# zhoujoey/ORB-SLAM3-Mac

Hardware: AMD Instinct MI355X
Metric: ORB extract+match frames/sec (higher is better)
Workload: dtype u8; 1 GPU; vga: synthetic 640x480 batch=1024 per GPU, 8-level pyramid, 1000 feats/frame, ORB extract + Hamming 2-NN match (Frame.cc:1146) + SearchForInitialization (ORBmatcher.cc:710) vs successor frame; pipelines=1, matchers=side by side (two contexts), frames_total=1024

## Files before the change

include/orbhip.h:

```cpp
#ifndef ORBHIP_H
#define ORBHIP_H
#include <stddef.h>
#include <stdint.h>
#ifdef __cplusplus
extern "C" {
#endif

#define ORBHIP_OK 0
#define ORBHIP_E_BADARG (-1)
#define ORBHIP_E_NODEVICE (-2)
#define ORBHIP_E_HIP (-3)
#define ORBHIP_E_CAPACITY (-4)
#define ORBHIP_E_ABORTED (-5)
#define ORBHIP_E_NOTSPD (-6)
#define ORBHIP_E_EMPTY (-7)

typedef struct {
    float x, y, size, angle, response;
    int32_t octave, class_id;
} orbhip_keypoint;

typedef struct orbhip_ctx orbhip_ctx;
typedef struct orbhip_extractor orbhip_extractor;

const char *orbhip_version(void);
const char *orbhip_last_error(void);

int orbhip_ctx_create(int device, void *stream, orbhip_ctx **out);
void orbhip_ctx_destroy(orbhip_ctx *ctx);
int orbhip_ctx_synchronize(orbhip_ctx *ctx);
int orbhip_ctx_wait_for(orbhip_ctx *ctx, orbhip_ctx *other);
int orbhip_ctx_check_status(orbhip_ctx *ctx);
void *orbhip_ctx_stream(orbhip_ctx *ctx);

int orbhip_extractor_create(orbhip_ctx *ctx, int nfeatures, float scale_factor, int nlevels,
                            int ini_th_fast, int min_th_fast, orbhip_extractor **out);
void orbhip_extractor_destroy(orbhip_extractor *ext);

int orbhip_extractor_levels(const orbhip_extractor *ext);
int orbhip_extractor_table(const orbhip_extractor *ext, int which, float *out);
int orbhip_extractor_features_per_level(const orbhip_extractor *ext, int *out);
int orbhip_extractor_umax(const orbhip_extractor *ext, int *out16);

int orbhip_extractor_reserve(orbhip_extractor *ext, int width, int height, int max_batch);
int orbhip_extractor_max_keypoints(const orbhip_extractor *ext);

int orbhip_extract_batch_device(orbhip_extractor *ext, const uint8_t *d_images, int width,
                                int height, size_t row_stride, size_t frame_stride, int batch,
                                int lap0, int lap1);
int orbhip_extractor_results(orbhip_extractor *ext, orbhip_keypoint **d_kp, uint8_t **d_desc,
                             int32_t **d_count, int32_t **d_mono_index);
int orbhip_extract_batch_host(orbhip_extractor *ext, const uint8_t *h_images, int width, int height,
                              size_t row_stride, size_t frame_stride, int batch, int lap0, int lap1,
                              orbhip_keypoint *kp_out, uint8_t *desc_out, int cap,
                              int32_t *count_out, int32_t *mono_out);
int orbhip_extract_batch_host_view(orbhip_extractor *ext, const uint8_t *h_images, int width, int height, size_t row_stride,
                                   size_t frame_stride, int batch, int lap0, int lap1, const orbhip_keypoint **kp_view,
                                   const uint8_t **desc_view, int *row_capacity, const int32_t **count_view, const int32_t **mono_view);
int orbhip_extractor_blur_kernel(const orbhip_extractor *ext, int batch);

int orbhip_extractor_resize_band_rows(const orbhip_extractor *ext, int level);

int orbhip_extractor_last_frame(orbhip_extractor *ext, int frame, const orbhip_keypoint **d_kp, const uint8_t **d_desc,
                                const orbhip_keypoint **h_kp_view, const uint8_t **h_desc_view, int32_t *count, unsigned long long *generation);

int orbhip_extractor_level_dims(const orbhip_extractor *ext, int level, int *w, int *h);
int orbhip_extractor_get_pyramid_level(orbhip_extractor *ext, int frame, int level, int padded,
                                       uint8_t *h_out, size_t out_stride);
int orbhip_extractor_get_pyramid_padded(orbhip_extractor *ext, int frame, uint8_t *const *levels_out, const size_t *strides);
int orbhip_extractor_get_blurred_level(orbhip_extractor *ext, int frame, int level,
                                       uint8_t *h_out, size_t out_stride);
int orbhip_extractor_get_fast_candidates(orbhip_extractor *ext, int frame, int level,
                                         int32_t *xs, int32_t *ys, int32_t *scores, int cap,
                                         int32_t *n_out);
int orbhip_extractor_get_level_keypoints(orbhip_extractor *ext, int frame, int level,
                                         orbhip_keypoint *out, int cap, int32_t *n_out);

int orbhip_extractor_set_graph_mode(orbhip_extractor *ext, int enable);

#define ORBHIP_STAGE_PYRAMID 0
#define ORBHIP_STAGE_FAST_CELLS 1
#define ORBHIP_STAGE_BLUR 2
#define ORBHIP_STAGE_OCTREE 3
#define ORBHIP_STAGE_DESC 4
#define ORBHIP_STAGE_ASSEMBLE 5
#define ORBHIP_STAGE_COUNT 6
int orbhip_extractor_set_profiling(orbhip_extractor *ext, int enable);
int orbhip_extractor_stage_ms(orbhip_extractor *ext, float *ms_out );

int orbhip_descriptor_distance(const uint8_t *a32, const uint8_t *b32);

int orbhip_match_bf2nn_device(orbhip_ctx *ctx, const uint8_t *d_descA, const int32_t *d_nA,
                              size_t strideA, const uint8_t *d_descB, const int32_t *d_nB,
                              size_t strideB, int pairs, int max_n, double ratio,
                              int32_t *d_idx2, int32_t *d_dist2, uint8_t *d_accept);

int orbhip_search_for_initialization_device(orbhip_ctx *ctx,
        const orbhip_keypoint *d_kpA, const uint8_t *d_descA, const int32_t *d_nA,
        const orbhip_keypoint *d_kpB, const uint8_t *d_descB, const int32_t *d_nB,
        int pairs, int max_n, size_t frame_stride_kp , float min_x, float min_y,
        float max_x, float max_y, int window_size, float nn_ratio, int check_orientation,
        float *d_prev_matched, int32_t *d_matches12, int32_t *d_nmatches);

int orbhip_prev_matched_init_device(orbhip_ctx *ctx, const orbhip_keypoint *d_kp, size_t frame_stride_kp,
                                    int frames, int max_n, float *d_prev_matched);

typedef struct orbhip_proj_query {
    float u, v, radius, ur, angle;
    int32_t min_level, max_level, has_obs;
} orbhip_proj_query;
int orbhip_search_by_projection_device(orbhip_ctx *ctx, const orbhip_proj_query *d_q, const uint8_t *d_desc_q,
                                       const int32_t *d_nq, int max_q, const orbhip_keypoint *d_kp,
                                       const uint8_t *d_desc, const float *d_u_right, const int32_t *d_n, int max_n,
                                       size_t frame_stride_kp, int pairs, float min_x, float min_y, float max_x,
                                       float max_y, int th_high, int check_orientation, int32_t *d_train_match,
                                       int32_t *d_nmatches);

int orbhip_search_local_map_device(orbhip_ctx *ctx, const orbhip_proj_query *d_q, const uint8_t *d_desc_q,
                                   const int32_t *d_nq, int max_q, const orbhip_keypoint *d_kp,
                                   const uint8_t *d_desc, const float *d_u_right, const int32_t *d_n, int max_n,
                                   size_t frame_stride_kp, int pairs, float min_x, float min_y, float max_x,
                                   float max_y, int th_high, float nn_ratio, int32_t *d_train_match,
                                   int32_t *d_nmatches);

int orbhip_search_by_projection_rig_device(orbhip_ctx *ctx, int mode, const orbhip_proj_query *d_q, const uint8_t *d_desc_q,
                                           const int32_t *d_nq, int max_q, const orbhip_keypoint *d_kp, const uint8_t *d_desc,
                                           const int32_t *d_n, const int32_t *d_nleft, const int32_t *d_mirror, int max_n,
                                           size_t frame_stride_kp, int pairs, float min_x, float min_y, float max_x, float max_y,
                                           int th_high, float nn_ratio, int check_orientation, int32_t *d_train_match,
// ... 398 lines not shown
```

orb-slam3-mac_amd/csrc/orb_kernels.hip:

```cpp
#include "orb_internal.h"
#include "wave_dpp.h"
#include <mutex>
#include <vector>
#include <cstdio>
#include <cstdlib>

#define WAVE 64

__device__ __forceinline__ int wave_incl_scan(int v) { return wave_scan_add_dpp(v); }

__device__ __forceinline__ int block_excl_scan256(int v, int *wsum, int *total)
{
    const int lane = threadIdx.x & (WAVE - 1), wid = threadIdx.x >> 6;
    int inc = wave_incl_scan(v);
    if (lane == WAVE - 1) wsum[wid] = inc;
    __syncthreads();
    int base = 0;
#pragma unroll
    for (int w = 0; w < 4; w++) {
        int s = wsum[w];
        if (w < wid) base += s;
    }
    *total = wsum[0] + wsum[1] + wsum[2] + wsum[3];
    __syncthreads();
// ... 754 lines not shown
    const long fair = total / (8 * nblocks);
    const int cmax = runs ? 8 : 4;
    F.chunk = chunk_env > 0 ? chunk_env : (int)(fair < 1 ? 1 : fair > cmax ? cmax : fair);
    if (runs && nld == 4) hipLaunchKernelGGL(k_fast_runs<4>, dim3((unsigned)nblocks), dim3(64), lds, s, F);
    else if (runs) hipLaunchKernelGGL(k_fast_runs<6>, dim3((unsigned)nblocks), dim3(64), lds, s, F);
    else if (F.small_cells) hipLaunchKernelGGL((k_fast_cells<3, 24, 2>), dim3((unsigned)nblocks), dim3(64), lds, s, F);
    else hipLaunchKernelGGL((k_fast_cells<5, 32, 5>), dim3((unsigned)nblocks), dim3(64), lds, s, F);
}
const void *orb_fast_cells_func(int small) { return small ? reinterpret_cast<const void *>(k_fast_cells<3, 24, 2>) : reinterpret_cast<const void *>(k_fast_cells<5, 32, 5>); }

struct OctLds {
    uint32_t *cc;
    int *ord;
    int *by_ord;
    int *excl;
    int *posbase;
    int *newpos;
    uint32_t *best;
};

int orb_octree_nc(const OrbParams &P)
{
    int nc = 0;
    for (int l = 0; l < P.nlevels; l++) { const int a = P.lv[l].quota + 16, b = 4 * P.lv[l].n_ini + 4; nc = a > nc ? a : nc; nc = b > nc ? b : nc; }
    return nc;
}

size_t orb_octree_lds_bytes(int nc)
{
    return (size_t)nc * 4 * (6 + 4 + 6) + 64;
}

__device__ __forceinline__ int oct_quadrant(uint32_t key, uint32_t b0, uint32_t b1)
{
    const int x0 = b0 & 0xFFFF, y0 = b0 >> 16, x1 = b1 & 0xFFFF, y1 = b1 >> 16;
    const int mx = x0 + ((x1 - x0 + 1) >> 1), my = y0 + ((y1 - y0 + 1) >> 1);
    const int kx = ORB_KEY_X(key), ky = ORB_KEY_Y(key);
    return (kx < mx ? 0 : 1) + (ky < my ? 0 : 2);
}

#define OCT_KR 8
#ifdef OCT_PROF
__device__ long long g_oct_prof[8];
#define OCT_T(i) do { if (blockIdx.x == 0 && threadIdx.x == 0) { const long long t_ = clock64(); g_oct_prof[i] += t_ - t_prev; t_prev = t_; } } while (0)
extern "C" int orbhip_debug_oct_prof(long long *out8, int reset)
{
    if (out8 && hipMemcpyFromSymbol(out8, HIP_SYMBOL(g_oct_prof), 64) != hipSuccess) return -1;
    if (reset) { long long z[8] = {0}; if (hipMemcpyToSymbol(HIP_SYMBOL(g_oct_prof), z, 64) != hipSuccess) return -1; }
    return 0;
}
#else
#define OCT_T(i) do { } while (0)
#endif
__device__ __forceinline__ int oct_gather(const OrbParams &P, const OrbLevel &L, int frame, int lvl, uint32_t *smem, int NC, int *wsum,
                                          uint32_t (&rk)[OCT_KR], uint32_t *keys)
{
    const int tid = threadIdx.x;
    const uint32_t *ccount = P.cell_count + (size_t)frame * P.cells_per_frame + L.cell_base;
    const uint32_t *clist = P.cell_list + (size_t)frame * P.cell_list_frame_stride + (size_t)L.cell_base * L.cell_cap;
    const int ncells = L.ncols * L.nrows;
    int running = 0;
    if (ncells + 1 <= 16 * NC) {
        int *coff = reinterpret_cast<int *>(smem);
        for (int c0 = 0; c0 < ncells; c0 += 256) {
            const int c = c0 + tid;
            const int n = c < ncells ? min((int)ccount[c], L.cell_cap) : 0;
            int total;
            const int off = running + block_excl_scan256(n, wsum, &total);
            if (c < ncells) coff[c] = off;
            running += total;
        }
        if (tid == 0) coff[ncells] = running;
        __syncthreads();
        if (running > L.key_cap) { if (tid == 0) atomicExch(P.status, ORBHIP_E_CAPACITY); running = L.key_cap; }
        const int K0 = running;
        auto fetch = [&](int k) {
            int lo = 0, hi = ncells;
            while (hi - lo > 1) { const int mid = (lo + hi) >> 1; if (coff[mid] <= k) lo = mid; else hi = mid; }
            return clist[(size_t)lo * L.cell_cap + (k - coff[lo])];
        };
#pragma unroll
        for (int i = 0; i < OCT_KR; i++) { const int k = tid + 256 * i; rk[i] = k < K0 ? fetch(k) : 0u; }
#pragma unroll
        for (int i = 0; i < OCT_KR; i++) { const int k = tid + 256 * i; if (k < K0) keys[k] = rk[i]; }
        for (int k = tid + 256 * OCT_KR; k < K0; k += 256) keys[k] = fetch(k);
        __syncthreads();
    } else {
        for (int c0 = 0; c0 < ncells; c0 += 256) {
            const int c = c0 + tid;
            const int n = c < ncells ? (int)ccount[c] : 0;
            int total;
            const int off = running + block_excl_scan256(n, wsum, &total);
            for (int i = 0; i < n; i++)
                if (off + i < L.key_cap) keys[off + i] = clist[(size_t)c * L.cell_cap + i];
            running += total;
        }
        if (running > L.key_cap) { if (tid == 0) atomicExch(P.status, ORBHIP_E_CAPACITY); running = L.key_cap; }
        __syncthreads();
        __threadfence_block();
#pragma unroll
        for (int i = 0; i < OCT_KR; i++) { const int k = tid + 256 * i; rk[i] = k < running ? keys[k] : 0u; }
    }
    if (tid == 0) P.lvl_ncand[frame * P.nlevels + lvl] = running;
    return running;
}

__device__ __forceinline__ void oct_output(const OrbParams &P, const OrbLevel &L, int frame, int lvl, uint32_t *best, int size, int K,
                                           const uint32_t (&rk)[OCT_KR], const int (&rn)[OCT_KR], const uint32_t *keys, const uint16_t *node_of,
                                           long long &t_prev)
{
    const int tid = threadIdx.x;
    int32_t *count_out = P.lvl_count + frame * P.nlevels + lvl;
    for (int i = tid; i < size; i += 256) best[i] = 0;
    __syncthreads();
#pragma unroll
    for (int i = 0; i < OCT_KR; i++)
        if (tid + 256 * i < K) atomicMax(&best[rn[i]], ((uint32_t)ORB_KEY_S(rk[i]) << 20) | (uint32_t)(0xFFFFF - (tid + 256 * i)));
    for (int k = tid + 256 * OCT_KR; k < K; k += 256)
        atomicMax(&best[node_of[k]], ((uint32_t)ORB_KEY_S(keys[k]) << 20) | (uint32_t)(0xFFFFF - k));
    __syncthreads();
    OCT_T(3);
    uint32_t *out = P.lvl_kp + (size_t)frame * P.kps_per_frame + L.kp_base;
    int nout = size;
    if (nout > L.kp_cap) { if (tid == 0) atomicExch(P.status, ORBHIP_E_CAPACITY); nout = L.kp_cap; }
    uint16_t *perm = P.lvl_perm + (size_t)frame * P.kps_per_frame + L.kp_base;
    for (int i = tid; i < nout; i += 256) out[i] = keys[0xFFFFF - (best[i] & 0xFFFFF)];
    if (P.batch < ORB_PERM_MIN_BATCH) { if (tid == 0) *count_out = nout; return; }
    __syncthreads();
    for (int i = tid; i < nout; i += 256) { const uint32_t ki = out[i]; best[i] = ((uint32_t)(ORB_KEY_Y(ki) >> 5) << 16) | (uint32_t)ORB_KEY_X(ki); }
    __syncthreads();
    for (int i = tid; i < nout; i += 256) {
        const uint32_t si = best[i];
        int rank = 0;
        for (int j = 0; j < nout; j++) { const uint32_t sj = best[j]; rank += (sj < si) || (sj == si && j < i); }
        perm[rank] = (uint16_t)i;
    }
    if (tid == 0) *count_out = nout;
    OCT_T(4);
}

__device__ __forceinline__ void oct_iterative(const OrbParams &P, const int lvl, const int frame)
{
    extern __shared__ uint32_t smem[];
    __shared__ int wsum[8];
    __shared__ int s_size, s_front, s_nexpand, s_rstar, s_T, s_nproc;
    const int tid = threadIdx.x;
    long long t_prev = 0;
#ifdef OCT_PROF
    t_prev = clock64();
#endif
    const OrbLevel &L = P.lv[lvl];
    const int N = L.quota;
    const int NC = P.oct_nc;
    uint32_t *box0 = smem, *box1 = smem + NC, *cnt = smem + 2 * NC;
    uint32_t *nbox0 = smem + 3 * NC, *nbox1 = smem + 4 * NC, *ncnt = smem + 5 * NC;
    OctLds S;
    {
        uint32_t *p = smem + 6 * NC;
        S.cc = p; p += 4 * NC;
        S.ord = (int *)p; p += NC; S.by_ord = (int *)p; p += NC; S.excl = (int *)p; p += NC;
        S.posbase = (int *)p; p += NC; S.newpos = (int *)p; p += NC; S.best = p; p += NC;
    }
    uint32_t *keys = P.keys + (size_t)frame * P.keys_per_frame + L.key_base;
    uint16_t *node_of = P.node_of + (size_t)frame * P.keys_per_frame + L.key_base;
    uint32_t rk[OCT_KR]; int rn[OCT_KR];
    int32_t *count_out = P.lvl_count + frame * P.nlevels + lvl;
    const int K = oct_gather(P, L, frame, lvl, smem, NC, wsum, rk, keys);
#pragma unroll
    for (int i = 0; i < OCT_KR; i++) rn[i] = 0;
    if (K == 0) { if (tid == 0) *count_out = 0; return; }
    __syncthreads();
    __threadfence_block();
    OCT_T(0);
    const int n_ini = L.n_ini;
    const int H = (L.h - ORB_MINB) - ORB_MINB;
    for (int i = tid; i < NC; i += 256) { cnt[i] = 0; ncnt[i] = 0; }
    __syncthreads();
#pragma unroll
    for (int i = 0; i < OCT_KR; i++)
        if (tid + 256 * i < K) {
            const int r = (int)__fdiv_rn((float)ORB_KEY_X(rk[i]), L.hx);
            rn[i] = r;
            atomicAdd(&ncnt[r], 1u);
        }
    for (int k = tid + 256 * OCT_KR; k < K; k += 256) {
        const int r = (int)__fdiv_rn((float)ORB_KEY_X(keys[k]), L.hx);
        node_of[k] = (uint16_t)r;
        atomicAdd(&ncnt[r], 1u);
// ... 117 lines not shown
                const int nch = (q[0] > 0) + (q[1] > 0) + (q[2] > 0) + (q[3] > 0);
                const int base = T - (S.excl[o] + nch);
                S.posbase[p] = base;
                const uint32_t b0 = box0[p], b1 = box1[p];
                const int x0 = b0 & 0xFFFF, y0 = b0 >> 16, x1 = b1 & 0xFFFF, y1 = b1 >> 16;
                const int mx = x0 + ((x1 - x0 + 1) >> 1), my = y0 + ((y1 - y0 + 1) >> 1);
                int pos = base, nexp = 0;
                for (int qd = 3; qd >= 0; qd--) {
                    if (q[qd]) {
                        const int cx0 = (qd & 1) ? mx : x0, cx1 = (qd & 1) ? x1 : mx;
                        const int cy0 = (qd & 2) ? my : y0, cy1 = (qd & 2) ? y1 : my;
                        nbox0[pos] = (uint32_t)cx0 | ((uint32_t)cy0 << 16);
                        nbox1[pos] = (uint32_t)cx1 | ((uint32_t)cy1 << 16);
                        ncnt[pos] = q[qd];
                        nexp += q[qd] > 1;
                        pos++;
                    }
                }
                if (nexp) atomicAdd(&s_nexpand, nexp);
            } else {
                const int np = S.newpos[p];
                nbox0[np] = box0[p]; nbox1[np] = box1[p]; ncnt[np] = cnt[p];
            }
        }
        __syncthreads();
        auto relabel = [&](uint32_t key, int p) {
            const int o = S.ord[p];
            if (o >= 0 && o <= rstar) {
                const int qd = oct_quadrant(key, box0[p], box1[p]);
                const uint32_t *q = &S.cc[4 * p];
                int r = 0;
                for (int j = 3; j > qd; j--) r += q[j] > 0;
                return S.posbase[p] + r;
            }
            return S.newpos[p];
        };
#pragma unroll
        for (int i = 0; i < OCT_KR; i++) if (tid + 256 * i < K) rn[i] = relabel(rk[i], rn[i]);
        for (int k = tid + 256 * OCT_KR; k < K; k += 256) node_of[k] = (uint16_t)relabel(keys[k], node_of[k]);
        __syncthreads();
        const int new_size = T + (size - nproc);
        const int nexpand = s_nexpand;
        { uint32_t *t; t = box0; box0 = nbox0; nbox0 = t; t = box1; box1 = nbox1; nbox1 = t; t = cnt; cnt = ncnt; ncnt = t; }
        const int old_size = size;
        size = new_size; front = T;
#ifdef OCT_PROF
        if (blockIdx.x == 0 && tid == 0) g_oct_prof[5] += 1;
#endif
        if (new_size >= N || new_size == old_size) break;
        if (!final_phase && new_size + 3 * nexpand > N) final_phase = true;
    }
    __syncthreads();
    OCT_T(2);
    oct_output(P, L, frame, lvl, S.best, size, K, rk, rn, keys, node_of, t_prev);
}

__global__ __launch_bounds__(256) void k_octree(OrbParams P)
{
    const int lvl = blockIdx.x / P.batch;
    oct_iterative(P, lvl, blockIdx.x - lvl * P.batch);
}

#define OCT_DMAX_LIMIT 7
#define OCT_TAB_NODE_WORDS 9
__host__ __device__ __forceinline__ int oct_tab_off(int n_ini, int d) { return n_ini * (((1 << (2 * d)) - 1) / 3); }

int orb_octree_dmax(const OrbParams &P)
{
    int n_ini = 1;
    for (int l = 0; l < P.nlevels; l++) n_ini = P.lv[l].n_ini > n_ini ? P.lv[l].n_ini : n_ini;
    int d = 0;
    while (d < OCT_DMAX_LIMIT && (long)oct_tab_off(n_ini, d + 2) <= (long)(16 - OCT_TAB_NODE_WORDS) * P.oct_nc) d++;
    return d >= 2 ? d : 0;
}

__device__ __forceinline__ uint32_t oct_path(uint32_t key, const OrbLevel &L, int H, int D)
{
    const int kx = ORB_KEY_X(key), ky = ORB_KEY_Y(key);
    const int r = min((int)__fdiv_rn((float)kx, L.hx), L.n_ini - 1);
    int x0 = (int)__fmul_rn(L.hx, (float)r), x1 = (int)__fmul_rn(L.hx, (float)(r + 1)), y0 = 0, y1 = H;
    uint32_t path = (uint32_t)r;
    for (int d = 0; d < D; d++) {
        const int mx = x0 + ((x1 - x0 + 1) >> 1), my = y0 + ((y1 - y0 + 1) >> 1);
        const bool qx = kx >= mx, qy = ky >= my;
        x0 = qx ? mx : x0; x1 = qx ? x1 : mx; y0 = qy ? my : y0; y1 = qy ? y1 : my;
        path = (path << 2) | (uint32_t)((qx ? 1 : 0) + (qy ? 2 : 0));
    }
    return path;
}

__global__ __launch_bounds__(256) void k_octree_tab(OrbParams P)
{
    extern __shared__ uint32_t smem[];
    __shared__ int wsum[8];
    __shared__ int s_nz[OCT_DMAX_LIMIT + 1], s_mu[OCT_DMAX_LIMIT + 1];
    __shared__ int s_front, s_rstar;
    const int tid = threadIdx.x;
    long long t_prev = 0;
#ifdef OCT_PROF
    t_prev = clock64();
#endif
    const int lvl = blockIdx.x / P.batch;
    const int frame = blockIdx.x - lvl * P.batch;
    const OrbLevel &L = P.lv[lvl];
    const int N = L.quota, NC = P.oct_nc, D = P.oct_dmax, n_ini = L.n_ini;
    const int H = (L.h - ORB_MINB) - ORB_MINB;
    uint32_t *cnt = smem, *ncnt = smem + NC, *tix = smem + 2 * NC, *ntix = smem + 3 * NC;
// ... 124 lines not shown
        __syncthreads();
        const int rstar = s_rstar;
        const int Tn = excl[rstar] + nchild(by_ord[rstar]), nproc = rstar + 1;
        {
            int run = 0;
            for (int p0 = 0; p0 < size; p0 += 256) {
                const int p = p0 + tid;
                const int surv = (p < size && !(ord[p] >= 0 && ord[p] <= rstar)) ? 1 : 0;
                int tot;
                const int e = run + block_excl_scan256(surv, wsum, &tot);
                if (p < size && surv) newpos[p] = Tn + e;
                run += tot;
            }
        }
        for (int p = tid; p < size; p += 256) {
            const int o = ord[p];
            if (o >= 0 && o <= rstar) {
                const uint32_t raw4 = 4 * (tix[p] & 0x7FFFFFFu);
                const uint32_t *q = ctab + raw4;
                int pos = Tn - (excl[o] + nchild(p));
                for (int qd = 3; qd >= 0; qd--)
                    if (q[qd]) { ncnt[pos] = q[qd]; ntix[pos] = ((uint32_t)(dcur + 1) << 27) | (raw4 + qd); pos++; }
            } else {
                const int np = newpos[p];
                ncnt[np] = cnt[p]; ntix[np] = tix[p];
            }
        }
        __syncthreads();
        { uint32_t *t; t = cnt; cnt = ncnt; ncnt = t; t = tix; tix = ntix; ntix = t; }
        const int old_size = size;
        size = Tn + (size - nproc); front = Tn; dcur++;
#ifdef OCT_PROF
        if (blockIdx.x == 0 && tid == 0) g_oct_prof[5] += 1;
#endif
        if (size >= N || size == old_size) break;
    }
    {
        const int Ef = oct_tab_off(n_ini, dcur + 1);
        for (int i = tid; i < Ef; i += 256) tab[i] = 0xFFFFFFFFu;
        __syncthreads();
        for (int p = tid; p < size; p += 256) { const uint32_t tx = tix[p]; tab[oct_tab_off(n_ini, (int)(tx >> 27)) + (tx & 0x7FFFFFFu)] = (uint32_t)p; }
        __syncthreads();
        auto node = [&](uint32_t path) {
            uint32_t nd = 0;
            for (int d = 0; d <= dcur; d++) { const uint32_t v = tab[oct_tab_off(n_ini, d) + (path >> (2 * (D - d)))]; if (v != 0xFFFFFFFFu) nd = v; }
            return (int)nd;
        };
#pragma unroll
        for (int i = 0; i < OCT_KR; i++) if (tid + 256 * i < K) rn[i] = node((uint32_t)rn[i]);
        for (int k = tid + 256 * OCT_KR; k < K; k += 256) node_of[k] = (uint16_t)node(oct_path(keys[k], L, H, D));
    }
    __syncthreads();
    OCT_T(2);
    oct_output(P, L, frame, lvl, best, size, K, rk, rn, keys, node_of, t_prev);
}

__global__ __launch_bounds__(256) void k_octree_redo(OrbParams P)
{
    __shared__ unsigned long long s_todo;
    const int tid = threadIdx.x, total = P.nlevels * P.batch, base = blockIdx.x * 64;
    if (tid < 64) {
        const int w = base + tid, lvl = w / P.batch;
        const bool f = w < total && P.lvl_count[(w - lvl * P.batch) * P.nlevels + lvl] < 0;
        const unsigned long long m = __ballot(f);
        if (tid == 0) s_todo = m;
    }
    __syncthreads();
    unsigned long long todo = s_todo;
    while (todo) {
        const int w = base + __ffsll((long long)todo) - 1, lvl = w / P.batch;
        todo &= todo - 1;
        oct_iterative(P, lvl, w - lvl * P.batch);
        __syncthreads();
    }
}

const void *orb_octree_func(int which)
{
    return which == 0 ? reinterpret_cast<const void *>(k_octree) : which == 1 ? reinterpret_cast<const void *>(k_octree_tab) : reinterpret_cast<const void *>(k_octree_redo);
}

void orb_launch_octree(const OrbParams &P, hipStream_t s, int parts)
{
    const size_t lds = orb_octree_lds_bytes(P.oct_nc);
    const int lists = P.nlevels * P.batch;
    if (P.oct_dmax <= 0) { hipLaunchKernelGGL(k_octree, dim3(lists), dim3(256), lds, s, P); return; }
    if (parts & 1) hipLaunchKernelGGL(k_octree_tab, dim3(lists), dim3(256), lds, s, P);
    if (parts & 2) hipLaunchKernelGGL(k_octree_redo, dim3((lists + 63) / 64), dim3(256), lds, s, P);
}

#define BL_TW 64
#define BL_TH 32
#define BL_ROWS (BL_TH + 6)
#define BL_IPD 20
__device__ __forceinline__ int reflect101(int p, int n)
{
    if (p < 0) p = -p;
    if (p >= n) p = 2 * n - 2 - p;
    return p;
}

__device__ __forceinline__ uint32_t bl_load4(const uint8_t *row, int x, int w)
{
    if (x >= 0 && x + 3 < w) return *reinterpret_cast<const uint32_t *>(row + x);
    uint32_t v = 0;
#pragma unroll
    for (int j = 0; j < 4; j++) {
// ... 583 lines not shown
```

orb-slam3-mac_amd/csrc/orbhip_api.hip:

```cpp
#include "orb_internal.h"
#include "ctx_internal.h"
#include <cmath>
#include <cfloat>
#include <cstdio>
#include <cstdlib>
#include <cstring>
#include <string>
#include <vector>
#include <mutex>
#include <set>
#include <utility>

static thread_local std::string g_last_error;
extern "C" const char *orbhip_last_error(void) { return g_last_error.c_str(); }
extern "C" const char *orbhip_version(void) { return "orbhip 0.1 (gfx950)"; }

#define HIP_TRY(expr)                                                                   \
    do {                                                                                \
        hipError_t _e = (expr);                                                         \
        if (_e != hipSuccess) {                                                         \
            g_last_error = std::string(#expr) + ": " + hipGetErrorString(_e);           \
            return ORBHIP_E_HIP;                                                        \
        }                                                                               \
    } while (0)
// ... 1114 lines not shown
}

extern "C" int orbhip_debug_octree(orbhip_extractor *e, int level, int nframes, const int32_t *offs, const int32_t *xs, const int32_t *ys,
                                   const int32_t *scores, int form, uint32_t *out_keys, int cap, int32_t *out_counts, int32_t *out_redo)
{
    if (!e || !e->max_batch || level < 0 || level >= e->nlevels || nframes < 1 || nframes > e->max_batch || !offs || !out_keys || !out_counts ||
        form < 0 || form > 1 || cap < 0) return ORBHIP_E_BADARG;
    if (form == 1 && e->oct_dmax_tab <= 0) { g_last_error = "the table form of the octree cannot run at this geometry"; return ORBHIP_E_BADARG; }
    OrbParams P = e->P;
    const OrbLevel &L = P.lv[level];
    P.batch = nframes; P.oct_dmax = form ? e->oct_dmax_tab : 0;
    std::vector<uint32_t> count((size_t)nframes * P.cells_per_frame, 0), list((size_t)nframes * P.cell_list_frame_stride, 0);
    for (int f = 0; f < nframes; f++) {
        if (offs[f + 1] < offs[f] || offs[f + 1] - offs[f] > L.key_cap) return ORBHIP_E_CAPACITY;
        for (int i = offs[f]; i < offs[f + 1]; i++) {
            if (xs[i] < 0 || xs[i] >= L.w - 2 * ORB_MINB || ys[i] < 0 || ys[i] >= L.h - 2 * ORB_MINB || scores[i] < 0 || scores[i] > 255) return ORBHIP_E_BADARG;
            const int c = std::min(ys[i] / L.hcell, L.nrows - 1) * L.ncols + std::min(xs[i] / L.wcell, L.ncols - 1);
            uint32_t &n = count[(size_t)f * P.cells_per_frame + L.cell_base + c];
            if ((int)n >= L.cell_cap) return ORBHIP_E_CAPACITY;
            list[(size_t)f * P.cell_list_frame_stride + ((size_t)L.cell_base + c) * L.cell_cap + n++] = ORB_PACK_KEY(xs[i], ys[i], scores[i]);
        }
    }
    HIP_TRY(hipSetDevice(e->ctx->device));
    hipStream_t s = e->ctx->stream;
    HIP_TRY(hipStreamSynchronize(s));
    HIP_TRY(hipMemcpy(P.cell_count, count.data(), sizeof(uint32_t) * count.size(), hipMemcpyHostToDevice));
    HIP_TRY(hipMemcpy(P.cell_list, list.data(), sizeof(uint32_t) * list.size(), hipMemcpyHostToDevice));
    std::vector<int32_t> cnt((size_t)nframes * P.nlevels);
    orb_launch_octree(P, s, 1);
    HIP_TRY(hipGetLastError());
    HIP_TRY(hipStreamSynchronize(s));
    if (out_redo) {
        HIP_TRY(hipMemcpy(cnt.data(), P.lvl_count, sizeof(int32_t) * cnt.size(), hipMemcpyDeviceToHost));
        for (int f = 0; f < nframes; f++) out_redo[f] = cnt[(size_t)f * P.nlevels + level] < 0 ? 1 : 0;
    }
    if (form) orb_launch_octree(P, s, 2);
    HIP_TRY(hipGetLastError());
    HIP_TRY(hipStreamSynchronize(s));
    HIP_TRY(hipMemcpy(cnt.data(), P.lvl_count, sizeof(int32_t) * cnt.size(), hipMemcpyDeviceToHost));
    int32_t st = 0;
    HIP_TRY(hipMemcpy(&st, P.status, sizeof(st), hipMemcpyDeviceToHost));
    if (st) { HIP_TRY(hipMemset(P.status, 0, sizeof(int32_t))); return st; }
    for (int f = 0; f < nframes; f++) {
        const int n = cnt[(size_t)f * P.nlevels + level];
        out_counts[f] = n;
        if (n < 0) return ORBHIP_E_HIP;
        const int m = std::min(n, cap);
        if (m > 0) HIP_TRY(hipMemcpy(out_keys + (size_t)f * cap, P.lvl_kp + (size_t)f * P.kps_per_frame + L.kp_base, sizeof(uint32_t) * m, hipMemcpyDeviceToHost));
    }
    e->last_batch = 0;
    return ORBHIP_OK;
}

extern "C" int orbhip_extractor_get_level_keypoints(orbhip_extractor *e, int frame, int level, orbhip_keypoint *out,
                                                    int cap, int32_t *n_out)
{
    if (!e || level < 0 || level >= e->nlevels || frame < 0 || frame >= e->last_batch || !n_out) return ORBHIP_E_BADARG;
    const OrbParams &P = e->P;
    const OrbLevel &L = P.lv[level];
    HIP_TRY(hipSetDevice(e->ctx->device));
    HIP_TRY(hipStreamSynchronize(e->ctx->stream));
    int32_t n = 0;
    HIP_TRY(hipMemcpy(&n, P.lvl_count + frame * P.nlevels + level, sizeof(n), hipMemcpyDeviceToHost));
    *n_out = n;
    int m = std::min(n, cap);
    if (m > 0 && out) {
        std::vector<uint32_t> k(m); std::vector<float> a(m);
        const size_t off = (size_t)frame * P.kps_per_frame + L.kp_base;
        HIP_TRY(hipMemcpy(k.data(), P.lvl_kp + off, sizeof(uint32_t) * m, hipMemcpyDeviceToHost));
        HIP_TRY(hipMemcpy(a.data(), P.lvl_angle + off, sizeof(float) * m, hipMemcpyDeviceToHost));
        for (int i = 0; i < m; i++) {
            out[i].x = (float)(ORB_KEY_X(k[i]) + ORB_MINB); out[i].y = (float)(ORB_KEY_Y(k[i]) + ORB_MINB);
            out[i].size = L.size; out[i].angle = a[i]; out[i].response = (float)ORB_KEY_S(k[i]);
            out[i].octave = level; out[i].class_id = -1;
        }
    }
    return ORBHIP_OK;
}
```

orb-slam3-mac_amd/python/orbhip.py:

```python
import ctypes as C
import os
import numpy as np

try:
    import torch
except Exception:
    torch = None

_HERE = os.path.dirname(os.path.abspath(__file__))
LIB_DIR = os.path.join(os.path.dirname(_HERE), "lib")
LIB_PATH = os.path.join(LIB_DIR, "liborbhip.so")
SYNTH_PATH = os.path.join(LIB_DIR, "libsynth.so")

if not os.path.exists(LIB_PATH):
    raise ImportError(
        "liborbhip.so not built: run `python -c 'import __graft_entry__ as g; g.build()'` "
        "(there is no CPU fallback for the HIP path)")

lib = C.CDLL(LIB_PATH)

OK, E_BADARG, E_NODEVICE, E_HIP, E_CAPACITY, E_ABORTED, E_NOTSPD, E_EMPTY = 0, -1, -2, -3, -4, -5, -6, -7
STAGES = ["pyramid", "fast_cells", "blur", "octree", "desc", "assemble"]

KP_DTYPE = np.dtype([("x", "<f4"), ("y", "<f4"), ("size", "<f4"), ("angle", "<f4"),
                     ("response", "<f4"), ("octave", "<i4"), ("class_id", "<i4")])
assert KP_DTYPE.itemsize == 28

vp, ci, cf, cd, sz = C.c_void_p, C.c_int, C.c_float, C.c_double, C.c_size_t
lib.orbhip_version.restype = C.c_char_p
lib.orbhip_last_error.restype = C.c_char_p
lib.orbhip_ctx_create.argtypes = [ci, vp, C.POINTER(vp)]
lib.orbhip_ctx_destroy.argtypes = [vp]
lib.orbhip_ctx_synchronize.argtypes = [vp]
lib.orbhip_ctx_stream.argtypes = [vp]
lib.orbhip_ctx_stream.restype = vp
lib.orbhip_extractor_create.argtypes = [vp, ci, cf, ci, ci, ci, C.POINTER(vp)]
lib.orbhip_extractor_destroy.argtypes = [vp]
lib.orbhip_extractor_levels.argtypes = [vp]
lib.orbhip_extractor_table.argtypes = [vp, ci, vp]
lib.orbhip_extractor_features_per_level.argtypes = [vp, vp]
lib.orbhip_extractor_umax.argtypes = [vp, vp]
lib.orbhip_extractor_reserve.argtypes = [vp, ci, ci, ci]
lib.orbhip_extractor_max_keypoints.argtypes = [vp]
lib.orbhip_extract_batch_device.argtypes = [vp, vp, ci, ci, sz, sz, ci, ci, ci]
lib.orbhip_extractor_results.argtypes = [vp, C.POINTER(vp), C.POINTER(vp), C.POINTER(vp), C.POINTER(vp)]
lib.orbhip_extract_batch_host.argtypes = [vp, vp, ci, ci, sz, sz, ci, ci, ci, vp, vp, ci, vp, vp]
lib.orbhip_extractor_level_dims.argtypes = [vp, ci, C.POINTER(ci), C.POINTER(ci)]
lib.orbhip_extractor_get_pyramid_level.argtypes = [vp, ci, ci, ci, vp, sz]
lib.orbhip_extractor_get_blurred_level.argtypes = [vp, ci, ci, vp, sz]
lib.orbhip_extractor_get_pyramid_padded.argtypes = [vp, ci, vp, vp]
lib.orbhip_extractor_get_fast_candidates.argtypes = [vp, ci, ci, vp, vp, vp, ci, C.POINTER(C.c_int32)]
lib.orbhip_extractor_get_level_keypoints.argtypes = [vp, ci, ci, vp, ci, C.POINTER(C.c_int32)]
lib.orbhip_extractor_set_profiling.argtypes = [vp, ci]
lib.orbhip_extractor_set_graph_mode.argtypes = [vp, ci]
lib.orbhip_extractor_stage_ms.argtypes = [vp, vp]
lib.orbhip_descriptor_distance.argtypes = [vp, vp]
lib.orbhip_match_bf2nn_device.argtypes = [vp, vp, vp, sz, vp, vp, sz, ci, ci, cd, vp, vp, vp]
lib.orbhip_search_for_initialization_device.argtypes = [vp, vp, vp, vp, vp, vp, vp, ci, ci, sz, cf, cf, cf, cf, ci, cf, ci,
                                                        vp, vp, vp]
lib.orbhip_ctx_check_status.argtypes = [vp]
lib.orbhip_ctx_wait_for.argtypes = [vp, vp]
lib.orbhip_extractor_blur_kernel.argtypes = [vp, ci]
lib.orbhip_extractor_blur_kernel.restype = ci
lib.orbhip_extractor_resize_band_rows.argtypes = [vp, ci]
lib.orbhip_extractor_resize_band_rows.restype = ci
if hasattr(lib, "orbhip_debug_octree"):
    lib.orbhip_debug_octree.argtypes = [vp, ci, ci, vp, vp, vp, vp, ci, vp, ci, vp, vp]
lib.orbhip_prev_matched_init_device.argtypes = [vp, vp, sz, ci, ci, vp]
lib.orbhip_search_by_projection_device.argtypes = [vp, vp, vp, vp, ci, vp, vp, vp, vp, ci, sz, ci, cf, cf, cf, cf, ci, ci, vp, vp]
lib.orbhip_search_local_map_device.argtypes = [vp, vp, vp, vp, ci, vp, vp, vp, vp, ci, sz, ci, cf, cf, cf, cf, ci, cf, vp, vp]


class OrbHipError(RuntimeError):
    def __init__(self, code, where):
        self.code = code
        super().__init__("%s failed: %d (%s)" % (where, code, lib.orbhip_last_error().decode()))


def _chk(rc, where):
    if rc != OK:
        raise OrbHipError(rc, where)


class Context:
    def __init__(self, device=0, stream=None):
        h = vp()
        _chk(lib.orbhip_ctx_create(device, stream, C.byref(h)), "orbhip_ctx_create")
        self.h = h

    def synchronize(self):
        _chk(lib.orbhip_ctx_synchronize(self.h), "orbhip_ctx_synchronize")

    def check_status(self):
        _chk(lib.orbhip_ctx_check_status(self.h), "orbhip_ctx_check_status")

    def wait_for(self, other):
        _chk(lib.orbhip_ctx_wait_for(self.h, other.h), "orbhip_ctx_wait_for")

    @property
    def stream(self):
        return lib.orbhip_ctx_stream(self.h)

    def close(self):
        if self.h:
            lib.orbhip_ctx_destroy(self.h)
            self.h = None


class Extractor:

    def __init__(self, ctx, nfeatures=1000, scale_factor=1.2, nlevels=8, ini_th=20, min_th=7):
        h = vp()
        _chk(lib.orbhip_extractor_create(ctx.h, nfeatures, scale_factor, nlevels, ini_th, min_th, C.byref(h)),
             "orbhip_extractor_create")
        self.h, self.ctx, self.nlevels = h, ctx, nlevels

    def close(self):
        if self.h:
            lib.orbhip_extractor_destroy(self.h)
            self.h = None

    def table(self, which):
        out = np.zeros(self.nlevels, np.float32)
        _chk(lib.orbhip_extractor_table(self.h, which, out.ctypes.data), "orbhip_extractor_table")
        return out

    def features_per_level(self):
        out = np.zeros(self.nlevels, np.int32)
        _chk(lib.orbhip_extractor_features_per_level(self.h, out.ctypes.data), "features_per_level")
        return out

    def umax(self):
        out = np.zeros(16, np.int32)
        _chk(lib.orbhip_extractor_umax(self.h, out.ctypes.data), "umax")
        return out

    def reserve(self, w, h, batch):
        _chk(lib.orbhip_extractor_reserve(self.h, w, h, batch), "orbhip_extractor_reserve")

    @property
    def max_keypoints(self):
        return lib.orbhip_extractor_max_keypoints(self.h)

    def blur_kernel(self, batch):
        return ("k_blur", "k_blur_rows", "k_blur_mfma")[lib.orbhip_extractor_blur_kernel(self.h, int(batch))]

    def resize_band_rows(self, level):
        return lib.orbhip_extractor_resize_band_rows(self.h, int(level))

    def debug_octree(self, level, lists, form):
        offs = np.zeros(len(lists) + 1, np.int32)
        offs[1:] = np.cumsum([len(l[0]) for l in lists])
        xs, ys, ss = (np.ascontiguousarray(np.concatenate([np.asarray(l[k], np.int32) for l in lists] + [np.zeros(1, np.int32)])) for k in range(3))
        cap = int(max(len(l[0]) for l in lists)) + 16
        keys = np.zeros((len(lists), cap), np.uint32)
        counts, redo = np.zeros(len(lists), np.int32), np.zeros(len(lists), np.int32)
        _chk(lib.orbhip_debug_octree(self.h, int(level), len(lists), offs.ctypes.data, xs.ctypes.data, ys.ctypes.data, ss.ctypes.data,
                                     {"iterative": 0, "table": 1}[form], keys.ctypes.data, cap, counts.ctypes.data, redo.ctypes.data),
             "orbhip_debug_octree")
        kept = [np.stack([k & 0xFFF, (k >> 12) & 0xFFF, k >> 24], 1).astype(np.int32) for k in (keys[f, :counts[f]] for f in range(len(lists)))]
        return kept, redo.tolist()

    def set_graph_mode(self, on):
        _chk(lib.orbhip_extractor_set_graph_mode(self.h, 1 if on else 0), "orbhip_extractor_set_graph_mode")

    def set_profiling(self, on):
        _chk(lib.orbhip_extractor_set_profiling(self.h, 1 if on else 0), "set_profiling")

    def stage_ms(self):
        out = np.zeros(len(STAGES), np.float32)
        _chk(lib.orbhip_extractor_stage_ms(self.h, out.ctypes.data), "stage_ms")
        return dict(zip(STAGES, out.tolist()))

    def extract_host(self, images, lap=(0, 1000)):
        img = np.ascontiguousarray(images, np.uint8)
        if img.ndim == 2:
            img = img[None]
        B, H, W = img.shape
        self.reserve(W, H, B)
        cap = self.max_keypoints
        kp = np.zeros((B, cap), KP_DTYPE)
        desc = np.zeros((B, cap, 32), np.uint8)
        cnt = np.zeros(B, np.int32)
        mono = np.zeros(B, np.int32)
        _chk(lib.orbhip_extract_batch_host(self.h, img.ctypes.data, W, H, W, W * H, B, lap[0], lap[1],
                                           kp.ctypes.data, desc.ctypes.data, cap, cnt.ctypes.data, mono.ctypes.data),
             "orbhip_extract_batch_host")
        return [(kp[f, :cnt[f]].copy(), desc[f, :cnt[f]].copy(), int(mono[f])) for f in range(B)]

    def extract_device(self, d_ptr, w, h, row_stride, frame_stride, batch, lap=(0, 1000)):
        _chk(lib.orbhip_extract_batch_device(self.h, d_ptr, w, h, row_stride, frame_stride, batch, lap[0], lap[1]),
             "orbhip_extract_batch_device")

    def results_device(self):
        a, b, c, d = vp(), vp(), vp(), vp()
        _chk(lib.orbhip_extractor_results(self.h, C.byref(a), C.byref(b), C.byref(c), C.byref(d)), "results")
        return a.value, b.value, c.value, d.value

    def level_dims(self, level):
        w, h = ci(), ci()
        _chk(lib.orbhip_extractor_level_dims(self.h, level, C.byref(w), C.byref(h)), "level_dims")
        return w.value, h.value

    def pyramid_level(self, frame, level, padded=False):
        w, h = self.level_dims(level)
        if padded:
            w, h = w + 38, h + 38
        out = np.zeros((h, w), np.uint8)
        _chk(lib.orbhip_extractor_get_pyramid_level(self.h, frame, level, 1 if padded else 0, out.ctypes.data, w),
             "get_pyramid_level")
        return out

    def pyramid_padded(self, frame):
        outs = [np.zeros((h + 38, w + 38), np.uint8) for w, h in (self.level_dims(l) for l in range(self.nlevels))]
# ... 784 lines not shown
```

Measured before the change: 333,400 frames/s.

## Replace quadratic rank-sort of octree keypoints with row-bucket counting sort

In the octree output stage, the keypoint permutation was computed by an O(n^2) rank count over all kept keypoints. It now writes winners directly from each candidate's node (removing a gather pass), builds a histogram of keypoints per 32-pixel row band in shared memory, and scatters them into bucket order. Each keypoint is then ranked only within its own bucket. This is meant to cut the quadratic sort cost in the octree kernels at large batch, in exchange for extra shared-memory arrays, atomics, and use of a scratch buffer. A debug API for reading the permutation back is added.

```diff
diff --git a/include/orbhip.h b/include/orbhip.h
--- a/include/orbhip.h
+++ b/include/orbhip.h
@@ -75,6 +75,7 @@
                                          int32_t *n_out);
 int orbhip_extractor_get_level_keypoints(orbhip_extractor *ext, int frame, int level,
                                          orbhip_keypoint *out, int cap, int32_t *n_out);
+int orbhip_debug_octree_perm(orbhip_extractor *ext, int level, int frame, uint16_t *out, int cap, int32_t *n_out);
 
 int orbhip_extractor_set_graph_mode(orbhip_extractor *ext, int enable);
 
diff --git a/orb-slam3-mac_amd/csrc/orb_kernels.hip b/orb-slam3-mac_amd/csrc/orb_kernels.hip
--- a/orb-slam3-mac_amd/csrc/orb_kernels.hip
+++ b/orb-slam3-mac_amd/csrc/orb_kernels.hip
@@ -830,6 +830,7 @@
 #else
 #define OCT_T(i) do { } while (0)
 #endif
+#define OCT_TROWS 128
 __device__ __forceinline__ int oct_gather(const OrbParams &P, const OrbLevel &L, int frame, int lvl, uint32_t *smem, int NC, int *wsum,
                                           uint32_t (&rk)[OCT_KR], uint32_t *keys)
 {
@@ -883,13 +884,16 @@
     return running;
 }
 
-__device__ __forceinline__ void oct_output(const OrbParams &P, const OrbLevel &L, int frame, int lvl, uint32_t *best, int size, int K,
+__device__ __forceinline__ void oct_output(const OrbParams &P, const OrbLevel &L, int frame, int lvl, uint32_t *best, uint32_t *scratch, int size, int K,
                                            const uint32_t (&rk)[OCT_KR], const int (&rn)[OCT_KR], const uint32_t *keys, const uint16_t *node_of,
                                            long long &t_prev)
 {
+    __shared__ int s_hist[OCT_TROWS], s_arr[OCT_TROWS];
     const int tid = threadIdx.x;
     int32_t *count_out = P.lvl_count + frame * P.nlevels + lvl;
+    const bool do_perm = P.batch >= ORB_PERM_MIN_BATCH;
     for (int i = tid; i < size; i += 256) best[i] = 0;
+    if (tid < OCT_TROWS) { s_hist[tid] = 0; s_arr[tid] = 0; }
     __syncthreads();
 #pragma unroll
     for (int i = 0; i < OCT_KR; i++)
@@ -901,17 +905,45 @@
     uint32_t *out = P.lvl_kp + (size_t)frame * P.kps_per_frame + L.kp_base;
     int nout = size;
     if (nout > L.kp_cap) { if (tid == 0) atomicExch(P.status, ORBHIP_E_CAPACITY); nout = L.kp_cap; }
+    uint32_t *skey = scratch, *srt = scratch + P.oct_nc;
+    auto winner = [&](uint32_t key, int node, int k) {
+        if (node < nout && best[node] == (((uint32_t)ORB_KEY_S(key) << 20) | (uint32_t)(0xFFFFF - k))) {
+            out[node] = key;
+            if (do_perm) { const int ty = ORB_KEY_Y(key) >> 5; skey[node] = ((uint32_t)ty << 16) | (uint32_t)ORB_KEY_X(key); atomicAdd(&s_hist[ty], 1); }
+        }
+    };
+#pragma unroll
+    for (int i = 0; i < OCT_KR; i++) if (tid + 256 * i < K) winner(rk[i], rn[i], tid + 256 * i);
+    for (int k = tid + 256 * OCT_KR; k < K; k += 256) winner(keys[k], node_of[k], k);
+    if (!do_perm) { if (tid == 0) *count_out = nout; return; }
+    __syncthreads();
     uint16_t *perm = P.lvl_perm + (size_t)frame * P.kps_per_frame + L.kp_base;
-    for (int i = tid; i < nout; i += 256) out[i] = keys[0xFFFFF - (best[i] & 0xFFFFF)];
-    if (P.batch < ORB_PERM_MIN_BATCH) { if (tid == 0) *count_out = nout; return; }
+    const int lane = tid & (WAVE - 1);
+    const int h0 = s_hist[2 * lane], h1 = s_hist[2 * lane + 1];
+    const int st0 = wave_incl_scan(h0 + h1) - h0 - h1;
+    for (int i0 = 0; i0 < nout; i0 += 256) {
+        const int i = i0 + tid;
+        const uint32_t s = i < nout ? skey[i] : 0u;
+        const int ty = (int)(s >> 16) & (OCT_TROWS - 1);
+        const int a = __shfl(st0, ty >> 1), b = __shfl(h0, ty >> 1);
+        if (i < nout) {
+            const int at = a + ((ty & 1) ? b : 0) + atomicAdd(&s_arr[ty], 1);
+            if (at < nout) srt[at] = ((s & 0xFFFFu) << 16) | (uint32_t)i;
+        }
+    }
     __syncthreads();
-    for (int i = tid; i < nout; i += 256) { const uint32_t ki = out[i]; best[i] = ((uint32_t)(ORB_KEY_Y(ki) >> 5) << 16) | (uint32_t)ORB_KEY_X(ki); }
-    __syncthreads();
-    for (int i = tid; i < nout; i += 256) {
-        const uint32_t si = best[i];
-        int rank = 0;
-        for (int j = 0; j < nout; j++) { const uint32_t sj = best[j]; rank += (sj < si) || (sj == si && j < i); }
-        perm[rank] = (uint16_t)i;
+    for (int i0 = 0; i0 < nout; i0 += 256) {
+        const int i = i0 + tid;
+        const uint32_t s = i < nout ? skey[i] : 0u;
+        const int ty = (int)(s >> 16) & (OCT_TROWS - 1);
+        const int a = __shfl(st0, ty >> 1), b = __shfl(h0, ty >> 1);
+        if (i < nout) {
+            const int start = a + ((ty & 1) ? b : 0), n = min(s_hist[ty], nout - start);
+            const uint32_t mine = ((s & 0xFFFFu) << 16) | (uint32_t)i;
+            int rank = start;
+            for (int j = 0; j < n; j++) rank += srt[start + j] < mine ? 1 : 0;
+            if (rank < nout) perm[rank] = (uint16_t)i;
+        }
     }
     if (tid == 0) *count_out = nout;
     OCT_T(4);
@@ -1135,7 +1167,7 @@
     }
     __syncthreads();
     OCT_T(2);
-    oct_output(P, L, frame, lvl, S.best, size, K, rk, rn, keys, node_of, t_prev);
+    oct_output(P, L, frame, lvl, S.best, S.cc, size, K, rk, rn, keys, node_of, t_prev);
 }
 
 __global__ __launch_bounds__(256) void k_octree(OrbParams P)
@@ -1366,7 +1398,7 @@
     }
     __syncthreads();
     OCT_T(2);
-    oct_output(P, L, frame, lvl, best, size, K, rk, rn, keys, node_of, t_prev);
+    oct_output(P, L, frame, lvl, best, smem, size, K, rk, rn, keys, node_of, t_prev);
 }
 
 __global__ __launch_bounds__(256) void k_octree_redo(OrbParams P)
diff --git a/orb-slam3-mac_amd/csrc/orbhip_api.hip b/orb-slam3-mac_amd/csrc/orbhip_api.hip
--- a/orb-slam3-mac_amd/csrc/orbhip_api.hip
+++ b/orb-slam3-mac_amd/csrc/orbhip_api.hip
@@ -1190,6 +1190,21 @@
     return ORBHIP_OK;
 }
 
+extern "C" int orbhip_debug_octree_perm(orbhip_extractor *e, int level, int frame, uint16_t *out, int cap, int32_t *n_out)
+{
+    if (!e || !e->max_batch || level < 0 || level >= e->nlevels || frame < 0 || frame >= e->max_batch || !n_out || cap < 0) return ORBHIP_E_BADARG;
+    const OrbParams &P = e->P;
+    const OrbLevel &L = P.lv[level];
+    HIP_TRY(hipSetDevice(e->ctx->device));
+    HIP_TRY(hipStreamSynchronize(e->ctx->stream));
+    int32_t n = 0;
+    HIP_TRY(hipMemcpy(&n, P.lvl_count + frame * P.nlevels + level, sizeof(n), hipMemcpyDeviceToHost));
+    *n_out = n;
+    const int m = std::min(std::min(n, cap), L.kp_cap);
+    if (m > 0 && out) HIP_TRY(hipMemcpy(out, P.lvl_perm + (size_t)frame * P.kps_per_frame + L.kp_base, sizeof(uint16_t) * m, hipMemcpyDeviceToHost));
+    return ORBHIP_OK;
+}
+
 extern "C" int orbhip_extractor_get_level_keypoints(orbhip_extractor *e, int frame, int level, orbhip_keypoint *out,
                                                     int cap, int32_t *n_out)
 {
diff --git a/orb-slam3-mac_amd/python/orbhip.py b/orb-slam3-mac_amd/python/orbhip.py
--- a/orb-slam3-mac_amd/python/orbhip.py
+++ b/orb-slam3-mac_amd/python/orbhip.py
@@ -66,6 +66,8 @@
 lib.orbhip_extractor_resize_band_rows.restype = ci
 if hasattr(lib, "orbhip_debug_octree"):
     lib.orbhip_debug_octree.argtypes = [vp, ci, ci, vp, vp, vp, vp, ci, vp, ci, vp, vp]
+if hasattr(lib, "orbhip_debug_octree_perm"):
+    lib.orbhip_debug_octree_perm.argtypes = [vp, ci, ci, vp, ci, C.POINTER(C.c_int32)]
 lib.orbhip_prev_matched_init_device.argtypes = [vp, vp, sz, ci, ci, vp]
 lib.orbhip_search_by_projection_device.argtypes = [vp, vp, vp, vp, ci, vp, vp, vp, vp, ci, sz, ci, cf, cf, cf, cf, ci, ci, vp, vp]
 lib.orbhip_search_local_map_device.argtypes = [vp, vp, vp, vp, ci, vp, vp, vp, vp, ci, sz, ci, cf, cf, cf, cf, ci, cf, vp, vp]
@@ -160,6 +162,13 @@
              "orbhip_debug_octree")
         kept = [np.stack([k & 0xFFF, (k >> 12) & 0xFFF, k >> 24], 1).astype(np.int32) for k in (keys[f, :counts[f]] for f in range(len(lists)))]
         return kept, redo.tolist()
+
+    def debug_octree_perm(self, level, frame):
+        n = C.c_int32(0)
+        _chk(lib.orbhip_debug_octree_perm(self.h, int(level), int(frame), None, 0, C.byref(n)), "orbhip_debug_octree_perm")
+        out = np.zeros(max(n.value, 1), np.uint16)
+        _chk(lib.orbhip_debug_octree_perm(self.h, int(level), int(frame), out.ctypes.data, out.size, C.byref(n)), "orbhip_debug_octree_perm")
+        return out[:max(n.value, 0)]
 
     def set_graph_mode(self, on):
         _chk(lib.orbhip_extractor_set_graph_mode(self.h, 1 if on else 0), "orbhip_extractor_set_graph_mode")
```

After: 335,200 frames/s (median of 6 runs). No clear change (+0.6%).
